# spaceml-org/STARCOP

Measured on AMD Instinct MI355X. Metric: 512x512 hyperspectral tiles/sec (train fwd+bwd), higher is better.
Workload: dtype f32; 1 GPU; configs[1]: HyperSTARCOP U-Net (smp.Unet mobilenet_v2, 4ch mag1c+RGB) train step fwd+loss+bwd+Adam, 512x512 tiles, fp32 HIP kernels (3x3 convs: fp32 operands split exactly into 16-bit terms on the matrix cores, fp32 accumulation; see config.precision and DESIGN.md section 2); batch_per_gpu=16, global_batch=16, parallelism=dp1, hipgraph=False, precision=fp32

## Files before the change

starcop_amd/csrc/conv_bx3.hip:

```cpp
#include "sc_split.h"
#include "conv_sp_pack.h"
#include <cstdlib>
#include <type_traits>


namespace {

struct ConvXP {
  SrcD s0, s1;
  const uintx4* wpk;
  int N, H, W, Cout;
  float* out0; float* out1;
  int csplit, accum0, accum1;
  const float* add0; const float* add1;
  float* stats;
  int down0;
  const float* absmax;
  const float* xb0; const float* xb1;
  int xcdmap;
  const float* bnr_y; const float* bnr_cst; float* bnr_rows; float* bnr_absmax; int bnr_act;
};

static inline void set_bnr(ConvXP& p, const sc_bnr_args* b) {
  p.bnr_y = b ? b->y : nullptr; p.bnr_cst = b ? b->cst : nullptr; p.bnr_rows = b ? b->rows : nullptr;
// ... 1965 lines not shown
      if (nn > nlast) { nn = pn; yy = py; xx = px; }
    };
    if (n1 > nlast) { n1 = n; y1 = y0; x1 = x0; }
    int n2 = n1, y2 = y1, x2 = x1;
    advance_sat(n2, y2, x2);
    if (t_begin < t_end) {
      x_load(xr, n, y0 - 1, x0);
      dy_load(n, y0, x0);
      x_store(xr, y0 - 1, x0, rp);
      x_load(xr, n, y0 + 1, x0);
      dy_store(0, y0, x0);
      x_store(xr, y0 + 1, x0, rp + 2);
      dy_load(n1, y1, x1);
      x_load(xr, n1, y1 + 1, x1);
      __syncthreads();
    }
    for (long t = t_begin; t < t_end; ++t) {
      if (y0 >= 0) compute(rp, buf);
#pragma unroll
      for (int k = 0; k < NDY; ++k) {
        dy_store_item(k, buf ^ 1, y1, x1);
        dy_load_item(k, n2, y2, x2);
      }
#pragma unroll
      for (int k = 0; k < NXI; ++k) {
        x_store_item(xr, k, y1 + 1, x1, rp + 4);
        x_load_item(xr, k, n2, y2 + 1, x2);
      }
      __syncthreads();
      rp = (rp + 2) & 7;
      buf ^= 1;
      n = n1; y0 = y1; x0 = x1;
      n1 = n2; y1 = y2; x1 = x2;
      advance_sat(n2, y2, x2);
    }
  }
  constexpr bool RED = PIPE && (KP == 1 || 3 * NPAIR * 3072 <= NT * CIT * XCP / 2);
  constexpr int KPP = RED ? 1 : KP;
  if constexpr (RED && KP > 1) {
    float* red = reinterpret_cast<float*>(&s_x[0][0]);
    const int slot = pair + NPAIR * kh;
#pragma unroll
    for (int k = 1; k < KP; ++k) {
      if (kp == k) {
#pragma unroll
        for (int kw = 0; kw < 3; ++kw)
#pragma unroll
          for (int r = 0; r < 16; ++r) red[slot * 3072 + (kw * 16 + r) * 64 + lane] = acc[kw][r];
      }
      __syncthreads();
      if (kp == 0) {
#pragma unroll
        for (int kw = 0; kw < 3; ++kw)
#pragma unroll
          for (int r = 0; r < 16; ++r) acc[kw][r] += red[slot * 3072 + (kw * 16 + r) * 64 + lane];
      }
      if (k + 1 < KP) __syncthreads();
    }
    if (kp != 0) return;
  }
  if (NPAIR == 3 && !computing) return;
  const int ci = cit * CIT + wn * 32 + l31;
  const size_t plane = (size_t)p.CoP * p.CiP;
  float* pb = p.part + ((size_t)blockIdx.x * KPP + (RED ? 0 : kp)) * 9 * plane;
#pragma unroll
  for (int kw = 0; kw < 3; ++kw) {
#pragma unroll
    for (int r = 0; r < 16; ++r) {
      const int co = cot * COT + wm * 32 + (r & 3) + 8 * (r >> 2) + 4 * lhi;
      if (co < p.CoP && ci < p.CiP) pb[(kh * 3 + kw) * plane + (size_t)co * p.CiP + ci] = HF ? acc[kw][r] * hinv : acc[kw][r];
    }
  }
}


template <int CIN, bool BNB>
__global__ __launch_bounds__(256, CIN == 32 ? 2 : 3) void k_wgrad_thin_h(const WgradXP p) {
  constexpr int NCB = CIN / 16, SR = 4, RING = 12;
#ifndef SC_WTH_DYPAD
#define SC_WTH_DYPAD(CIN) ((CIN) == 16 ? 16 : 8)
#endif
#ifndef SC_WTH_XPAD
#define SC_WTH_XPAD 16
#endif
  constexpr int DYP = SR * 32 + SC_WTH_DYPAD(CIN);
  constexpr int XP = 40, XCP = RING * XP + SC_WTH_XPAD;
  constexpr int NDY = (16 * SR * 16) / 256;
  constexpr int XCNT = CIN * SR * 17;
  constexpr int NXI = (XCNT + 255) / 256;
  __shared__ __attribute__((aligned(16))) unsigned s_dy[2][2][16 * DYP / 2];
  __shared__ __attribute__((aligned(16))) unsigned s_x[2][CIN * XCP / 2];
  __shared__ __attribute__((aligned(16))) float s_ca[16 * SC_CST];
  __shared__ __attribute__((aligned(16))) float s_cb[CIN * 4];

  const int tid = threadIdx.x, lane = tid & 63, wave = tid >> 6;
  const int l15 = lane & 15, lg = lane >> 4;
  const int H = p.H, W = p.W;
  const float hsg = h_grad_scale(p.absmax);
  const float hsa = h_act_scale(p.xb0, p.xb1);
  const float hinv = 1.f / (hsg * hsa);

  for (int i = tid; i < 16 * SC_CST; i += 256) {
    const int ch = i / SC_CST, f = i % SC_CST;
    const float fs = (BNB ? (f >= 2 && f <= 4) : (f < 2)) ? hsg : 1.f;
    s_ca[i] = fs * ((p.dy.cst && p.dy.mode != SC_SRC_RAW && ch < p.Cout) ? p.dy.cst[(size_t)ch * SC_CST + f] : (f == 0 ? 1.f : 0.f));
  }
  for (int i = tid; i < CIN; i += 256) {
    float sc = 1.f, sh = 0.f;
    if (p.s0.cst && p.s0.mode != SC_SRC_RAW) { sc = p.s0.cst[(size_t)i * SC_CST]; sh = p.s0.cst[(size_t)i * SC_CST + 1]; }
    s_cb[i * 4] = sc * hsa; s_cb[i * 4 + 1] = sh * hsa;
    s_cb[i * 4 + 2] = h_lo(sc_act_lo(p.s0.act), hsa); s_cb[i * 4 + 3] = h_hi(sc_act_hi(p.s0.act), hsa);
  }

  floatx4 acc[9][NCB];
#pragma unroll
  for (int t = 0; t < 9; ++t)
#pragma unroll
    for (int cb = 0; cb < NCB; ++cb) acc[t][cb] = (floatx4){0.f, 0.f, 0.f, 0.f};

  const int tiles_x = (W + 31) >> 5, RS = (H + SR - 1) / SR, RSS = RS + 1;
  const long T = (long)p.N * tiles_x * RSS;
  const long t_begin = T * blockIdx.x / p.nsl, t_end = T * (blockIdx.x + 1) / p.nsl;
  const float dlo = sc_act_lo(p.dy.act) * (BNB ? 1.f : hsg), dhi = sc_act_hi(p.dy.act) * (BNB ? 1.f : hsg);
  const size_t HW = (size_t)H * W;
  const int up = p.s0.up, Ws = W >> up;
  const unsigned istr = (unsigned)((size_t)CIN * (H >> up) * Ws * 4);

  unsigned dyo[NDY], xo[NXI];
#pragma unroll
  for (int k = 0; k < NDY; ++k) {
    const int co = (tid + 256 * k) >> 6;
    dyo[k] = (unsigned)(co < p.Cout ? co : 0) * (unsigned)HW * 4u;
  }
#pragma unroll
  for (int k = 0; k < NXI; ++k) {
    int it = tid + 256 * k;
    if (it >= XCNT) it -= XCNT;
    xo[k] = (unsigned)((it / 17) >> 2) * (unsigned)((H >> up) * Ws) * 4u;
  }

  float dg[NDY][2], dv[BNB ? NDY : 1][2], xr[NXI][2];
  auto dy_load_item = [&](int k, int n, int y0, int x0) {
    const int it = tid + 256 * k;
    const int row = (it >> 4) & 3, col = 2 * (it & 15);
    const int y = y0 + row, x = x0 + col;
    const size_t io = (size_t)n * p.Cout * HW * 4;
    const unsigned off = dyo[k] + (unsigned)(((y >= 0 && y < H) ? y : 0) * W + ((x < W) ? x : 0)) * 4u;
    const float2 g = *reinterpret_cast<const float2*>(reinterpret_cast<const char*>(p.dy.x) + io + off);
    dg[k][0] = g.x; dg[k][1] = g.y;
    if (BNB) {
      const float2 a = *reinterpret_cast<const float2*>(reinterpret_cast<const char*>(p.dy.aux) + io + off);
      dv[k][0] = a.x; dv[k][1] = a.y;
    }
  };
  auto dy_store_item = [&](int k, int buf, int y0, int x0) {
    const int it = tid + 256 * k;
    const int co = it >> 6, row = (it >> 4) & 3, col = 2 * (it & 15);
    const int y = y0 + row, x = x0 + col;
    const bool ok = (co < p.Cout) && y >= 0 && y < H && x < W;
    const float4 c0 = *reinterpret_cast<const float4*>(&s_ca[co * SC_CST]);
    const float c4 = s_ca[co * SC_CST + 4];
    float v0, v1;
    if (BNB) {
      v0 = sc_pro_bnbwd(dg[k][0], dv[k][0], c0.x, c0.y, c0.z, c0.w, c4, dlo, dhi);
      v1 = sc_pro_bnbwd(dg[k][1], dv[k][1], c0.x, c0.y, c0.z, c0.w, c4, dlo, dhi);
    } else {
      v0 = sc_pro_affine(dg[k][0], c0.x, c0.y, dlo, dhi);
      v1 = sc_pro_affine(dg[k][1], c0.x, c0.y, dlo, dhi);
    }
    v0 = ok ? v0 : 0.f;
    v1 = ok ? v1 : 0.f;
    unsigned t0, t1;
    split2h(v0, v1, t0, t1);
    const int d = (co * DYP + row * 32 + col) >> 1;
    s_dy[buf][0][d] = t0; s_dy[buf][1][d] = t1;
  };
  auto x_load_item = [&](int k, int n, int R, int x0) {
    int it = tid + 256 * k;
    if (it >= XCNT) it -= XCNT;
    const int rc = it / 17, pr = it - rc * 17;
    const int rowi = rc & 3;
    const int y = R + rowi, x = x0 - 1 + 2 * pr;
    const int yc = (y >= 0 && y < H) ? y : 0;
    const int xa = (x >= 0 && x < W) ? x : 0, xb = (x + 1 < W) ? x + 1 : 0;
    const char* base = reinterpret_cast<const char*>(p.s0.x) + (size_t)n * istr;
    const unsigned ro = xo[k] + (unsigned)((yc >> up) * Ws) * 4u;
    xr[k][0] = *reinterpret_cast<const float*>(base + (ro + (unsigned)(xa >> up) * 4u));
    xr[k][1] = *reinterpret_cast<const float*>(base + (ro + (unsigned)(xb >> up) * 4u));
  };
  auto x_store_item = [&](int k, int R, int x0, int sl0) {
    int it = tid + 256 * k;
    if (it >= XCNT) it -= XCNT;
    const int rc = it / 17, pr = it - rc * 17;
    const int rowi = rc & 3, cil = rc >> 2;
    const int y = R + rowi, x = x0 - 1 + 2 * pr;
    const bool oky = (y >= 0) && (y < H);
    const float4 c = *reinterpret_cast<const float4*>(&s_cb[cil * 4]);
    float v0 = sc_pro_affine_h(xr[k][0], c.x, c.y, c.z, c.w);
    float v1 = sc_pro_affine_h(xr[k][1], c.x, c.y, c.z, c.w);
    v0 = (oky && x >= 0 && x < W) ? v0 : 0.f;
    v1 = (oky && x + 1 < W) ? v1 : 0.f;
    unsigned t0, t1;
    split2h<false>(v0, v1, t0, t1);
    int slot = sl0 + rowi;
    slot = slot >= RING ? slot - RING : slot;
    const int d = ((cil * XCP + slot * XP) >> 1) + pr;
    s_x[0][d] = t0; s_x[1][d] = t1;
  };
  auto ring = [](int v) { return v >= RING ? v - RING : v; };
  const unsigned opaque_zero = (unsigned)p.H >> 30;
  auto compute = [&](int rp, int buf) {
    const int r = wave;
    halfx8 A[2];
    const int da = (l15 * DYP + r * 32 + 8 * lg) >> 1;
#pragma unroll
    for (int tm = 0; tm < 2; ++tm) A[tm] = __builtin_bit_cast(halfx8, *reinterpret_cast<const uintx4*>(&s_dy[buf][tm][da]));
#pragma unroll
    for (int kh = 0; kh < 3; ++kh) {
      const int slot = ring(rp + r + kh);
#pragma unroll
      for (int cb = 0; cb < NCB; ++cb) {
        const int dx = (((cb * 16 + l15) * XCP + slot * XP) >> 1) + 4 * lg;
        halfx8 B[3][2];
#pragma unroll
        for (int tm = 0; tm < 2; ++tm) {
          const uintx4 X0 = *reinterpret_cast<const uintx4*>(&s_x[tm][dx]);
          const uintx4 X1v = *reinterpret_cast<const uintx4*>(&s_x[tm][dx + 4]);
          const unsigned X1 = X1v[0] | (X1v[1] & opaque_zero);
          uintx4 S1, S2;
          S1[0] = __builtin_amdgcn_alignbit(X0[1], X0[0], 16);
          S1[1] = __builtin_amdgcn_alignbit(X0[2], X0[1], 16);
          S1[2] = __builtin_amdgcn_alignbit(X0[3], X0[2], 16);
          S1[3] = __builtin_amdgcn_alignbit(X1, X0[3], 16);
          S2[0] = X0[1]; S2[1] = X0[2]; S2[2] = X0[3]; S2[3] = X1;
          B[0][tm] = __builtin_bit_cast(halfx8, X0);
          B[1][tm] = __builtin_bit_cast(halfx8, S1);
          B[2][tm] = __builtin_bit_cast(halfx8, S2);
        }
#pragma unroll
        for (int kw = 0; kw < 3; ++kw) {
          floatx4 c = acc[kh * 3 + kw][cb];
          c = __builtin_amdgcn_mfma_f32_16x16x32_f16(A[0], B[kw][1], c, 0, 0, 0);
          c = __builtin_amdgcn_mfma_f32_16x16x32_f16(A[1], B[kw][0], c, 0, 0, 0);
          c = __builtin_amdgcn_mfma_f32_16x16x32_f16(A[0], B[kw][0], c, 0, 0, 0);
          acc[kh * 3 + kw][cb] = c;
        }
      }
    }
  };

  const int nlast = p.N - 1;
  auto advance = [&](int& nn, int& yy, int& xx) {
    const int pn = nn, py = yy, px = xx;
    yy += SR;
    if (yy >= SR * RS) { yy = -SR; xx += 32; if (xx >= 32 * tiles_x) { xx = 0; ++nn; } }
    if (nn > nlast) { nn = pn; yy = py; xx = px; }
  };
  int n = 0, y0 = 0, x0 = 0;
  if (t_begin < t_end) {
    const int strip = (int)(t_begin / RSS), ty = (int)(t_begin - (long)strip * RSS);
    n = strip / tiles_x; x0 = (strip - n * tiles_x) * 32; y0 = (ty - 1) * SR;
  }
  n = __builtin_amdgcn_readfirstlane(n); y0 = __builtin_amdgcn_readfirstlane(y0); x0 = __builtin_amdgcn_readfirstlane(x0);
  int n1 = n, y1 = y0, x1 = x0;
  advance(n1, y1, x1);
  int n2 = n1, y2 = y1, x2 = x1;
  advance(n2, y2, x2);
  __syncthreads();
  int rp = 0, buf = 0;
  if (t_begin < t_end) {
#pragma unroll
    for (int k = 0; k < NXI; ++k) x_load_item(k, n, y0 - 1, x0);
#pragma unroll
    for (int k = 0; k < NDY; ++k) dy_load_item(k, n, y0, x0);
#pragma unroll
    for (int k = 0; k < NXI; ++k) { x_store_item(k, y0 - 1, x0, rp); x_load_item(k, n, y0 + 3, x0); }
#pragma unroll
    for (int k = 0; k < NDY; ++k) { dy_store_item(k, 0, y0, x0); dy_load_item(k, n1, y1, x1); }
#pragma unroll
    for (int k = 0; k < NXI; ++k) { x_store_item(k, y0 + 3, x0, rp + 4); x_load_item(k, n1, y1 + 1, x1); }
    __syncthreads();
  }
  for (long t = t_begin; t < t_end; ++t) {
    if (y0 >= 0) compute(rp, buf);
#pragma unroll
    for (int k = 0; k < NDY; ++k) {
      dy_store_item(k, buf ^ 1, y1, x1);
      dy_load_item(k, n2, y2, x2);
    }
    const int sl1 = ring(rp + 6);
#pragma unroll
    for (int k = 0; k < NXI; ++k) {
      x_store_item(k, y1 + 1, x1, sl1);
      x_load_item(k, n2, y2 + 1, x2);
    }
    __syncthreads();
    rp = ring(rp + 4);
    buf ^= 1;
    n = n1; y0 = y1; x0 = x1;
    n1 = n2; y1 = y2; x1 = x2;
    advance(n2, y2, x2);
  }
  float* red = reinterpret_cast<float*>(&s_x[0][0]);
  auto put = [&](int slot) {
#pragma unroll
    for (int tap = 0; tap < 9; ++tap)
#pragma unroll
      for (int cb = 0; cb < NCB; ++cb)
        *reinterpret_cast<floatx4*>(&red[(((slot * 9 + tap) * NCB + cb) * 64 + lane) * 4]) = acc[tap][cb];
  };
  auto take = [&](int slot) {
#pragma unroll
    for (int tap = 0; tap < 9; ++tap)
#pragma unroll
      for (int cb = 0; cb < NCB; ++cb) acc[tap][cb] += *reinterpret_cast<const floatx4*>(&red[(((slot * 9 + tap) * NCB + cb) * 64 + lane) * 4]);
  };
  if (wave >= 2) put(wave - 2);
  __syncthreads();
  if (wave < 2) take(wave);
  __syncthreads();
  if (wave == 1) put(0);
  __syncthreads();
  if (wave == 0) {
    take(0);
    const size_t plane = (size_t)16 * CIN;
    float* pb = p.part + (size_t)blockIdx.x * 9 * plane;
#pragma unroll
    for (int tap = 0; tap < 9; ++tap)
#pragma unroll
      for (int cb = 0; cb < NCB; ++cb)
#pragma unroll
        for (int r = 0; r < 4; ++r) pb[tap * plane + (size_t)(4 * lg + r) * CIN + cb * 16 + l15] = acc[tap][cb][r] * hinv;
  }
}

struct WgradXPlan { int wm, nci, kp, nsl, CoP, CiP, co_tiles, ci_tiles; };
WgradXPlan plan_wgrad_bx3(int N, int H, int W, int Cout, int Cin, bool allow96 = false) {
  WgradXPlan pl;
  pl.wm = Cout > 32 ? 2 : 1;
  pl.nci = Cin <= 32 ? 1 : 2;
  if (allow96 && pl.wm == 1 && Cin > 64 && Cin <= 96) pl.nci = 3;
  pl.kp = pl.nci * pl.wm == 3 ? 1 : 4 / (pl.nci * pl.wm);
  pl.CoP = (Cout + 31) / 32 * 32;
  pl.CiP = (Cin + 31) / 32 * 32;
  pl.co_tiles = (Cout + 32 * pl.wm - 1) / (32 * pl.wm);
  pl.ci_tiles = (Cin + 32 * pl.nci - 1) / (32 * pl.nci);
  const long T = (long)N * ((W + 31) / 32) * ((H + 1) / 2);
  const long tiles = (long)pl.co_tiles * pl.ci_tiles;
  const long nmax = T / 4 < 512 ? (T / 4 > 1 ? T / 4 : 1) : 512;
  auto cost = [&](long k) { return (double)((tiles * k + 255) / 256) * ((double)((T + k - 1) / k) + 6.0); };
  double best_cost = 1e30;
  for (long k = 1; k <= nmax; ++k) best_cost = cost(k) < best_cost ? cost(k) : best_cost;
  long best = 1;
  for (long k = 1; k <= nmax; ++k)
    if (cost(k) <= 1.03 * best_cost) { best = k; break; }
  long want = best;
  pl.nsl = (int)want;
  return pl;
}


struct PackDesc {
  const float* w; float* wpk;
  int Cout, Cin, ks, co_t, tflip, bx3;
  unsigned long long total;
};
static_assert(sizeof(PackDesc) == sizeof(sc_pack_desc), "sc_pack_desc layout");

__global__ __launch_bounds__(256) void k_pack_batch(const PackDesc* __restrict__ descs, const unsigned* __restrict__ starts, int n) {
  int lo = 0, hi = n - 1;
  while (lo < hi) {
    const int mid = (lo + hi + 1) >> 1;
    if (starts[mid] <= blockIdx.x) lo = mid; else hi = mid - 1;
  }
  const PackDesc d = descs[lo];
  const size_t i = (size_t)(blockIdx.x - starts[lo]) * 256 + threadIdx.x;
  if (i >= d.total) return;
  if (d.bx3 == SC_PACK_THIN16) { pack_thin_item(d.w, reinterpret_cast<unsigned short*>(d.wpk), i, d.Cout, d.Cin, d.tflip); return; }
  if (d.bx3 == SC_PACK_SPD) { spd_pack_item(d.w, reinterpret_cast<unsigned short*>(d.wpk), i, d.Cout, d.Cin, d.co_t, (d.tflip & 3) == 2, (d.tflip & 4) != 0, (d.tflip & 3) == 3 ? d.Cin - d.co_t : 0); return; }
  if (d.bx3 == SC_PACK_SP) { sp_pack_item(d.w, reinterpret_cast<unsigned short*>(d.wpk), i, d.Cout, d.co_t, d.Cin - d.co_t, (d.tflip & 4) != 0); return; }
  const int M = d.tflip ? d.Cin : d.Cout, K = d.tflip ? d.Cout : d.Cin;
  if (d.bx3 == SC_PACK_PW3) {
    const int nks = (K + 15) / 16;
    const int j = (int)(i % 8), lane = (int)((i / 8) % 64);
    const int ks = (int)((i / 512) % nks), cb = (int)(i / ((size_t)512 * nks));
    const int m = cb * 32 + (lane & 31), k = ks * 16 + 8 * (lane >> 5) + j;
    float v = 0.f;
    if (m < M && k < K) v = d.tflip ? d.w[(size_t)k * M + m] : d.w[(size_t)m * K + k];
    unsigned short t[3];
    split_filter(v, false, t);
    unsigned short* out = reinterpret_cast<unsigned short*>(d.wpk);
    for (int c = 0; c < 3; ++c) out[((((size_t)cb * nks + ks) * 3 + c) * 64 + lane) * 8 + j] = t[c];
    return;
  }
  const int taps = d.ks * d.ks;
  if (!d.bx3) {
    const int kc = d.ks == 3 ? 8 : 16;
    const int Kpad = (K + kc - 1) / kc * kc;
    const int col = (int)(i % d.co_t);
    size_t r = i / d.co_t;
    const int tap = (int)(r % taps); r /= taps;
    const int k = (int)(r % Kpad);
    const int m = (int)(r / Kpad) * d.co_t + col;
    float v = 0.f;
    if (m < M && k < K) v = d.tflip ? d.w[((size_t)k * M + m) * taps + (taps - 1 - tap)] : d.w[((size_t)m * K + k) * taps + tap];
    d.wpk[i] = v;
    return;
  }
  const int nchunk = (K + 15) / 16;
  size_t r = i;
  const int j = (int)(r % 8); r /= 8;
  const int col = (int)(r % d.co_t); r /= d.co_t;
  const int half = (int)(r % 2); r /= 2;
  const int kw = (int)(r % 3); r /= 3;
  const int kh = (int)(r % 3); r /= 3;
  const int chunk = (int)(r % nchunk);
  const int mt = (int)(r / nchunk);
  const int m = mt * d.co_t + col, k = chunk * 16 + half * 8 + j, tap = kh * 3 + kw;
  float v = 0.f;
  if (m < M && k < K) v = d.tflip ? d.w[((size_t)k * M + m) * 9 + (8 - tap)] : d.w[((size_t)m * K + k) * 9 + tap];
  unsigned short t[3];
  const bool hmode = d.bx3 == SC_TERMS_F16X2;
  const int nt = hmode ? 2 : d.bx3;
  split_filter(v, hmode, t);
  const size_t stage = ((size_t)mt * nchunk + chunk) * 3 + kh;
  unsigned short* out = reinterpret_cast<unsigned short*>(d.wpk);
  for (int c = 0; c < nt; ++c) out[((((stage * nt + c) * 3 + kw) * 2 + half) * d.co_t + col) * 8 + j] = t[c];
}

}

extern "C" size_t sc_packed_weight_floats_bx3(int Cout, int Cin, int co_t, int transpose_flip, int terms) {
  const int M = transpose_flip ? Cin : Cout, K = transpose_flip ? Cout : Cin;
  const size_t mt = (M + co_t - 1) / co_t, nchunk = (K + 15) / 16;
  return mt * nchunk * 3 * 6 * (size_t)(terms == SC_TERMS_F16X2 ? 2 : (terms >= 1 && terms <= 3 ? terms : 3)) * co_t * 4;
}

extern "C" int sc_pack_weights_bx3(const float* w, float* wpk, int Cout, int Cin, int co_t, int transpose_flip,
                                   int terms, sc_stream stream) {
  SC_REQUIRE(terms >= 1 && terms <= 4, "sc_pack_weights_bx3: terms must be 1, 2, 3 or SC_TERMS_F16X2 (got %d)", terms);
  SC_REQUIRE(w && wpk && Cout > 0 && Cin > 0, "sc_pack_weights_bx3: bad argument");
  SC_REQUIRE(co_t == 32 || co_t == 64, "sc_pack_weights_bx3: co_t must be 32 or 64 (got %d)", co_t);
  SC_REQUIRE(((uintptr_t)wpk & 15) == 0, "sc_pack_weights_bx3: destination must be 16-byte aligned");
  const int M = transpose_flip ? Cin : Cout, K = transpose_flip ? Cout : Cin;
  const int nchunk = (K + 15) / 16;
  const size_t total = (size_t)((M + co_t - 1) / co_t) * nchunk * 9 * 2 * co_t * 8;
  const int blocks = (int)((total + 255) / 256 > 4096 ? 4096 : (total + 255) / 256);
  hipLaunchKernelGGL(k_pack_weights_bx3, dim3(blocks), dim3(256), 0, (hipStream_t)stream, w,
                     reinterpret_cast<unsigned short*>(wpk), Cout, Cin, co_t, transpose_flip, nchunk,
                     terms == SC_TERMS_F16X2 ? 2 : terms, terms == SC_TERMS_F16X2 ? 1 : 0, total);
  SC_LAUNCH_OK("sc_pack_weights_bx3");
  return SC_OK;
}

extern "C" int sc_conv3x3_bx3(const sc_conv_args* a, sc_stream stream) {
  SC_REQUIRE(a != nullptr, "sc_conv3x3_bx3: null args");
  SC_REQUIRE(a->ks == 3, "sc_conv3x3_bx3: ks must be 3 (got %d)", a->ks);
  SC_REQUIRE(a->co_t == 32 || a->co_t == 64, "sc_conv3x3_bx3: co_t must be 32 or 64 (got %d)", a->co_t);
  SC_REQUIRE(a->nsrc == 1 || a->nsrc == 2, "sc_conv3x3_bx3: nsrc must be 1 or 2");
  const int C0 = a->src[0].C, C1 = a->nsrc == 2 ? a->src[1].C : 0;
  SC_REQUIRE(C0 > 0 && C1 >= 0 && (a->nsrc == 1 || (C0 % 16 == 0 && C1 > 0)),
             "sc_conv3x3_bx3: a concat needs the first source's channels to be a multiple of 16 (got %d,%d)", C0, C1);
  SC_REQUIRE(a->N > 0 && a->H > 0 && a->W > 0 && a->Cout > 0, "sc_conv3x3_bx3: bad shape");
  SC_REQUIRE(a->csplit > 0 && a->csplit <= a->Cout, "sc_conv3x3_bx3: bad csplit");
  SC_REQUIRE(a->csplit == a->Cout || (a->add0 == nullptr && a->add1 == nullptr), "sc_conv3x3_bx3: add tensors need a single output");
  SC_REQUIRE(((uintptr_t)a->wpk & 15) == 0, "sc_conv3x3_bx3: packed filters must be 16-byte aligned");
  for (int s = 0; s < a->nsrc; ++s) {
    SC_REQUIRE(a->src[s].up == 0 || (a->H % 2 == 0 && a->W % 2 == 0), "sc_conv3x3_bx3: upsampled source needs even H,W");
    SC_REQUIRE(a->src[s].up == 0 || a->src[s].up == 1, "sc_conv3x3_bx3: up must be 0 or 1");
    SC_REQUIRE(a->src[s].mode == SC_SRC_RAW || a->src[s].cst != nullptr, "sc_conv3x3_bx3: source %d needs constants", s);
    SC_REQUIRE(a->src[s].mode != SC_SRC_NORM, "sc_conv3x3_bx3: NORM sources are the stem's");
    SC_REQUIRE(a->src[s].mode != SC_SRC_BNBWD || a->src[s].aux != nullptr, "sc_conv3x3_bx3: BNBWD source needs aux");
    SC_REQUIRE(a->src[s].mode != SC_SRC_BNBWD || a->nsrc == 1, "sc_conv3x3_bx3: a BNBWD source cannot be part of a concat");
  }
  ConvXP p;
  p.s0 = to_srcd(a->src[0]);
  p.s1 = a->nsrc == 2 ? to_srcd(a->src[1]) : empty_srcd();
  p.wpk = reinterpret_cast<const uintx4*>(a->wpk); p.N = a->N; p.H = a->H; p.W = a->W; p.Cout = a->Cout;
  p.out0 = a->out0; p.out1 = a->out1; p.csplit = a->csplit; p.accum0 = a->accum0; p.accum1 = a->accum1;
  p.add0 = a->add0; p.add1 = a->add1; p.stats = a->stats;
  p.down0 = a->down0 ? 1 : 0;
  SC_REQUIRE(!p.down0 || (a->H % 2 == 0 && a->W % 2 == 0 && a->stats == nullptr && a->add0 == nullptr && a->add1 == nullptr),
             "sc_conv3x3_bx3: down0 (2x2-summed half-resolution out0) needs even H, W and no stats/add tensors");
  const int co_tiles = (a->Cout + a->co_t - 1) / a->co_t;
  dim3 grid(((a->W + 31) / 32) * ((a->H + 7) / 8), co_tiles, a->N);
  constexpr int xcdmap_env = 2;
  p.xcdmap = xcdmap_env >= 2 ? 2 : ((xcdmap_env && co_tiles > 1) ? 1 : 0);
  {
    constexpr long big_env = 0L;
    const long nkc = (C0 + C1 + 15) / 16;
    const long wbytes = (long)co_tiles * nkc * 3 * 6 * (a->terms == SC_TERMS_F16X2 || a->terms == 2 ? 2 : (a->terms == 1 ? 1 : 3)) * a->co_t * 16;
    if (xcdmap_env >= 2 && big_env > 0 && wbytes > big_env && (co_tiles >= 8 || co_tiles == 1 || co_tiles == 2 || co_tiles == 4)) p.xcdmap = 3;
  }
  if (p.xcdmap == 3) {
    const long total = (long)grid.x * a->N;
    const long slots = co_tiles >= 8 ? (long)((co_tiles + 7) / 8) * total : (total + (8 / co_tiles) - 1) / (8 / co_tiles);
    SC_REQUIRE(slots * 8 < (1L << 31), "sc_conv3x3_bx3: grid too large");
    grid = dim3((unsigned)(slots * 8));
  } else if (p.xcdmap) {
    const long pt8 = ((long)grid.x * a->N + 7) / 8 * 8;
    SC_REQUIRE(pt8 * co_tiles < (1L << 31), "sc_conv3x3_bx3: grid too large");
    grid = dim3((unsigned)(pt8 * co_tiles));
  }
  hipStream_t st = (hipStream_t)stream;
  const bool bnb = a->src[0].mode == SC_SRC_BNBWD;
  SC_REQUIRE(a->terms >= 0 && a->terms <= 4, "sc_conv3x3_bx3: terms must be 0 (= 3), 1, 2, 3 or SC_TERMS_F16X2 (got %d)", a->terms);
  p.absmax = a->absmax; p.xb0 = a->xbound[0]; p.xb1 = a->xbound[1];
  set_bnr(p, a->bnr);
  if (a->bnr) {
    SC_REQUIRE(bnb && a->bnr->y && a->bnr->cst && a->bnr->rows, "sc_conv3x3_bx3: bnr needs a BNBWD source and y / cst / rows");
    SC_REQUIRE(!a->accum0 && !a->add0 && !a->add1 && !a->stats, "sc_conv3x3_bx3: bnr: out0 must receive the complete gradient (no accum0 / add / stats)");
    SC_REQUIRE(a->csplit == a->Cout || a->csplit % a->co_t == 0, "sc_conv3x3_bx3: bnr: csplit must fall on a cout-tile boundary");
  }
#define SC_LAUNCH_BX3(NT, HF)                                                                                  \
  do {                                                                                                         \
    if (a->co_t == 64 && bnb) hipLaunchKernelGGL((k_conv3_bx3<2, true, NT, HF>), grid, dim3(256), 0, st, p);   \
    else if (a->co_t == 64) hipLaunchKernelGGL((k_conv3_bx3<2, false, NT, HF>), grid, dim3(256), 0, st, p);    \
    else if (bnb) hipLaunchKernelGGL((k_conv3_bx3<1, true, NT, HF>), grid, dim3(256), 0, st, p);               \
    else hipLaunchKernelGGL((k_conv3_bx3<1, false, NT, HF>), grid, dim3(256), 0, st, p);                       \
  } while (0)
  constexpr int ws_env = 1;
  static const int ws_env_min = [] { const char* e = getenv("STARCOP_BX3_WS_MINCHUNKS"); return e ? atoi(e) : 16; }();
  if (a->terms == 1) SC_LAUNCH_BX3(1, false); else if (a->terms == 2) SC_LAUNCH_BX3(2, false);
  else if (a->terms == SC_TERMS_F16X2 && ws_env && (C0 + C1 + 15) / 16 >= ws_env_min && (!bnb || a->src[0].C <= 256) && !a->bnr) {
    if (a->co_t == 64 && bnb) hipLaunchKernelGGL((k_conv3_ws<2, true>), grid, dim3(512), 0, st, p);
    else if (a->co_t == 64) hipLaunchKernelGGL((k_conv3_ws<2, false>), grid, dim3(512), 0, st, p);
    else if (bnb) hipLaunchKernelGGL((k_conv3_ws<1, true>), grid, dim3(512), 0, st, p);
    else hipLaunchKernelGGL((k_conv3_ws<1, false>), grid, dim3(512), 0, st, p);
  }
  else if (a->terms == SC_TERMS_F16X2) SC_LAUNCH_BX3(2, true); else SC_LAUNCH_BX3(3, false);
#undef SC_LAUNCH_BX3
  SC_LAUNCH_OK("sc_conv3x3_bx3");
  return SC_OK;
}

static bool wgrad3_pipe_reduces(const WgradXPlan& pl) {
  const int npair = pl.nci * pl.wm, cit = 32 * pl.nci, xcp = 8 * 40 + 8;
  return pl.kp == 1 || 3 * npair * 3072 <= 2 * cit * xcp / 2;
}

static size_t wgrad_bx3_workspace_of(const WgradXPlan& pl) {
  const size_t E = (size_t)9 * pl.CoP * pl.CiP;
  const int nparts = pl.nsl * pl.kp;
  return (size_t)nparts * E + sc_reduce_scratch_floats(nparts, E);
}
extern "C" size_t sc_wgrad_bx3_workspace_floats(int N, int H, int W, int Cout, int Cin) {
  const size_t a = wgrad_bx3_workspace_of(plan_wgrad_bx3(N, H, W, Cout, Cin, false));
  const size_t b = wgrad_bx3_workspace_of(plan_wgrad_bx3(N, H, W, Cout, Cin, true));
  return a > b ? a : b;
}

extern "C" int sc_conv3x3_wgrad_bx3(const sc_wgrad_args* a, sc_stream stream) {
  SC_REQUIRE(a != nullptr, "sc_conv3x3_wgrad_bx3: null args");
  SC_REQUIRE(a->ks == 3, "sc_conv3x3_wgrad_bx3: ks must be 3");
  SC_REQUIRE(a->nsrc == 1 || a->nsrc == 2, "sc_conv3x3_wgrad_bx3: nsrc must be 1 or 2");
  const int C0 = a->src[0].C, C1 = a->nsrc == 2 ? a->src[1].C : 0;
  SC_REQUIRE(C0 + C1 == a->Cin, "sc_conv3x3_wgrad_bx3: source channels (%d+%d) != Cin %d", C0, C1, a->Cin);
  SC_REQUIRE(a->dy.C == a->Cout, "sc_conv3x3_wgrad_bx3: dy channels %d != Cout %d", a->dy.C, a->Cout);
  SC_REQUIRE(a->dy.up == 0 && a->dy.mode != SC_SRC_NORM, "sc_conv3x3_wgrad_bx3: unsupported dy source");
  SC_REQUIRE(a->dy.mode != SC_SRC_BNBWD || a->dy.aux != nullptr, "sc_conv3x3_wgrad_bx3: BNBWD dy needs aux");
  SC_REQUIRE(a->N > 0 && a->H > 0 && a->W > 0 && a->Cout > 0 && a->Cin > 0, "sc_conv3x3_wgrad_bx3: bad shape");
  for (int s = 0; s < a->nsrc; ++s) {
    SC_REQUIRE(a->src[s].mode == SC_SRC_RAW || a->src[s].mode == SC_SRC_AFFINE, "sc_conv3x3_wgrad_bx3: input sources must be RAW or AFFINE");
    SC_REQUIRE(a->src[s].up == 0 || (a->src[s].up == 1 && a->H % 2 == 0 && a->W % 2 == 0), "sc_conv3x3_wgrad_bx3: upsampled source needs even H,W");
  }
  static const bool no96 = [] { const char* e = getenv("STARCOP_WGRAD96"); return e && atoi(e) == 0; }();
  constexpr int pipe_env = 1;
  bool pipe = pipe_env && a->terms == SC_TERMS_F16X2 && a->dy.mode == SC_SRC_BNBWD && a->W % 2 == 0 && (((uintptr_t)a->dy.x | (uintptr_t)a->dy.aux) & 7) == 0 &&
              (size_t)a->Cout * a->H * a->W * 4 < (1ull << 32);
  for (int s = 0; s < a->nsrc; ++s) pipe = pipe && (size_t)a->N * a->src[s].C * (a->H >> a->src[s].up) * (a->W >> a->src[s].up) * 4 < (1ull << 32);
  const WgradXPlan pl = plan_wgrad_bx3(a->N, a->H, a->W, a->Cout, a->Cin, pipe && !no96);
  const size_t need = sc_wgrad_bx3_workspace_floats(a->N, a->H, a->W, a->Cout, a->Cin);
  SC_REQUIRE(a->part_floats >= need, "sc_conv3x3_wgrad_bx3: workspace too small (%zu < %zu floats)", a->part_floats, need);
  WgradXP p;
  p.dy = to_srcd(a->dy); p.s0 = to_srcd(a->src[0]); p.s1 = a->nsrc == 2 ? to_srcd(a->src[1]) : empty_srcd();
  p.N = a->N; p.H = a->H; p.W = a->W; p.Cout = a->Cout; p.Cin = a->Cin; p.part = a->part;
  p.nsl = pl.nsl; p.CoP = pl.CoP; p.CiP = pl.CiP;
  dim3 grid(pl.nsl, pl.ci_tiles, pl.co_tiles);
  hipStream_t st = (hipStream_t)stream;
  SC_REQUIRE(a->terms >= 0 && a->terms <= 4, "sc_conv3x3_wgrad_bx3: terms must be 0 (= 3), 1, 2, 3 or SC_TERMS_F16X2 (got %d)", a->terms);
  p.absmax = a->absmax; p.xb0 = a->xbound[0]; p.xb1 = a->xbound[1];
  int nparts = pl.nsl * pl.kp;
#define SC_WGX(WM_, NT_, NCI_, HF_, PIPE_) hipLaunchKernelGGL((k_wgrad3_bx3<WM_, NT_, NCI_, HF_, PIPE_>), grid, dim3(768), 0, st, p)
#define SC_WGX_NT(NT_, HF_, PIPE_)                                   \
  do {                                                               \
    if constexpr (HF_ && PIPE_) { if (pl.nci == 3) { SC_WGX(1, NT_, 3, HF_, PIPE_); break; } }      \
    if (pl.wm == 2 && pl.nci == 2) SC_WGX(2, NT_, 2, HF_, PIPE_);    \
    else if (pl.wm == 2) SC_WGX(2, NT_, 1, HF_, PIPE_);              \
    else if (pl.nci == 2) SC_WGX(1, NT_, 2, HF_, PIPE_);             \
    else SC_WGX(1, NT_, 1, HF_, PIPE_);                              \
  } while (0)
  if (a->terms == 1) SC_WGX_NT(1, false, false); else if (a->terms == 2) SC_WGX_NT(2, false, false);
  else if (a->terms == SC_TERMS_F16X2) {
    if (pipe) { SC_WGX_NT(2, true, true); if (wgrad3_pipe_reduces(pl)) nparts = pl.nsl; } else SC_WGX_NT(2, true, false);
  }
  else SC_WGX_NT(3, false, false);
#undef SC_WGX_NT
#undef SC_WGX
  SC_LAUNCH_OK("sc_conv3x3_wgrad_bx3");
  return sc_wgrad_finish(a->part, nparts, 9, a->Cout, a->Cin, pl.CoP, pl.CiP, a->dw, st);
}

static int wgrad_thin16_slices(int N, int H, int W, int Cin) {
  const long T = (long)N * ((W + 31) / 32) * ((H + 3) / 4 + 1);
  const long full = Cin > 16 ? 512 : 768;
  return (int)(T < full ? T : full);
}

extern "C" size_t sc_wgrad_thin16_workspace_floats(int N, int H, int W, int Cout, int Cin) {
  (void)Cout;
  const size_t E = (size_t)9 * 16 * Cin;
  const int nparts = wgrad_thin16_slices(N, H, W, Cin);
  return (size_t)nparts * E + sc_reduce_scratch_floats(nparts, E);
}

extern "C" int sc_conv3x3_wgrad_thin16(const sc_wgrad_args* a, sc_stream stream) {
  SC_REQUIRE(a != nullptr && a->ks == 3 && a->nsrc == 1, "sc_conv3x3_wgrad_thin16: one source, ks = 3");
  SC_REQUIRE(a->Cout >= 1 && a->Cout <= 16 && (a->Cin == 16 || a->Cin == 32) && a->src[0].C == a->Cin && a->dy.C == a->Cout,
             "sc_conv3x3_wgrad_thin16: needs <= 16 output and 16 or 32 input channels (got %d, %d)", a->Cout, a->Cin);
  SC_REQUIRE(a->N > 0 && a->H > 0 && a->W > 0, "sc_conv3x3_wgrad_thin16: bad shape");
  SC_REQUIRE(a->terms == SC_TERMS_F16X2, "sc_conv3x3_wgrad_thin16: terms must be SC_TERMS_F16X2");
  SC_REQUIRE(a->dy.up == 0 && a->dy.mode != SC_SRC_NORM && (a->dy.mode != SC_SRC_BNBWD || a->dy.aux != nullptr), "sc_conv3x3_wgrad_thin16: unsupported dy source");
  SC_REQUIRE(a->dy.mode == SC_SRC_RAW || a->dy.cst != nullptr, "sc_conv3x3_wgrad_thin16: dy source needs constants");
  const sc_src& s = a->src[0];
  SC_REQUIRE((s.mode == SC_SRC_RAW || (s.mode == SC_SRC_AFFINE && s.cst != nullptr)), "sc_conv3x3_wgrad_thin16: input source must be RAW or AFFINE");
  SC_REQUIRE(s.up == 0 || (s.up == 1 && a->H % 2 == 0 && a->W % 2 == 0), "sc_conv3x3_wgrad_thin16: upsampled source needs even H, W");
  SC_REQUIRE((size_t)a->Cout * a->H * a->W * 4 < (1ull << 32) && (size_t)a->N * a->Cin * a->H * a->W * 4 < (1ull << 32),
             "sc_conv3x3_wgrad_thin16: tensors too large for 32-bit byte offsets");
  SC_REQUIRE(a->W % 2 == 0 && (((uintptr_t)a->dy.x | (uintptr_t)a->dy.aux) & 7) == 0, "sc_conv3x3_wgrad_thin16: needs an even width and 8-byte aligned gradient tensors");
  const size_t need = sc_wgrad_thin16_workspace_floats(a->N, a->H, a->W, a->Cout, a->Cin);
  SC_REQUIRE(a->part_floats >= need, "sc_conv3x3_wgrad_thin16: workspace too small (%zu < %zu floats)", a->part_floats, need);
  WgradXP p;
  p.absmax = a->absmax; p.xb0 = a->xbound[0]; p.xb1 = a->xbound[1];
  p.dy = to_srcd(a->dy); p.s0 = to_srcd(s); p.s1 = empty_srcd();
  p.N = a->N; p.H = a->H; p.W = a->W; p.Cout = a->Cout; p.Cin = a->Cin; p.part = a->part;
  p.nsl = wgrad_thin16_slices(a->N, a->H, a->W, a->Cin); p.CoP = 16; p.CiP = a->Cin;
  hipStream_t st = (hipStream_t)stream;
  const bool bnb = a->dy.mode == SC_SRC_BNBWD;
  dim3 grid(p.nsl);
  if (a->Cin == 16) { if (bnb) hipLaunchKernelGGL((k_wgrad_thin_h<16, true>), grid, dim3(256), 0, st, p); else hipLaunchKernelGGL((k_wgrad_thin_h<16, false>), grid, dim3(256), 0, st, p); }
  else              { if (bnb) hipLaunchKernelGGL((k_wgrad_thin_h<32, true>), grid, dim3(256), 0, st, p); else hipLaunchKernelGGL((k_wgrad_thin_h<32, false>), grid, dim3(256), 0, st, p); }
  SC_LAUNCH_OK("sc_conv3x3_wgrad_thin16");
  return sc_wgrad_finish(a->part, p.nsl, 9, a->Cout, a->Cin, 16, a->Cin, a->dw, st);
}

static int thin_steps(int Cout, int Cin, int transpose_flip) {
  const int K = transpose_flip ? Cout : Cin;
  if (transpose_flip && Cin == 32) return 16;
  return (9 * (K / 8) + 3) / 4 + ((!transpose_flip && K == 32) ? 16 : 0);
}

extern "C" size_t sc_packed_weight_floats_thin16(int Cout, int Cin, int transpose_flip) {
  return (size_t)thin_steps(Cout, Cin, transpose_flip) * 2 * 64 * 4;
}

static bool thin16_shape_ok(int Cout, int Cin, int transpose_flip) {
  const int M = transpose_flip ? Cin : Cout, K = transpose_flip ? Cout : Cin;
  if (transpose_flip && Cin == 32 && Cout == 16) return true;
  return M >= 1 && M <= 16 && (K == 16 || K == 32);
}

extern "C" int sc_pack_weights_thin16(const float* w, float* wpk, int Cout, int Cin, int transpose_flip, sc_stream stream) {
  SC_REQUIRE(w && wpk && ((uintptr_t)wpk & 15) == 0, "sc_pack_weights_thin16: bad pointer");
  SC_REQUIRE(thin16_shape_ok(Cout, Cin, transpose_flip), "sc_pack_weights_thin16: needs <= 16 output and 16 or 32 input channels (got %d, %d, flip %d)",
             Cout, Cin, transpose_flip);
  const size_t total = (size_t)thin_steps(Cout, Cin, transpose_flip) * 512;
  hipLaunchKernelGGL(k_pack_weights_thin, dim3((unsigned)((total + 255) / 256)), dim3(256), 0, (hipStream_t)stream, w,
                     reinterpret_cast<unsigned short*>(wpk), Cout, Cin, transpose_flip, total);
  SC_LAUNCH_OK("sc_pack_weights_thin16");
  return SC_OK;
}

extern "C" int sc_conv3x3_thin16(const sc_conv_args* a, sc_stream stream) {
  SC_REQUIRE(a != nullptr && a->ks == 3 && a->nsrc == 1, "sc_conv3x3_thin16: one source, ks = 3");
  const int Cin = a->src[0].C;
  if (a->down0) {
    const sc_src& s = a->src[0];
    SC_REQUIRE(Cin == 16 && a->Cout == 32 && a->csplit == 32 && s.mode == SC_SRC_BNBWD && s.aux && s.cst && s.up == 0,
               "sc_conv3x3_thin16(down0): needs a 16-channel BatchNorm-backward source and 32 output channels (got %d, %d)", Cin, a->Cout);
    SC_REQUIRE(a->H % 2 == 0 && a->W % 2 == 0 && a->N > 0 && a->N <= 65535 && a->out0 && !a->add0 && !a->add1 && !a->stats && !a->bnr && !a->out1,
               "sc_conv3x3_thin16(down0): even H, W; one output, no add / statistics / bnr epilogue");
    SC_REQUIRE(a->terms == SC_TERMS_F16X2 && ((uintptr_t)a->wpk & 15) == 0, "sc_conv3x3_thin16(down0): terms must be SC_TERMS_F16X2, filters 16-byte aligned");
    SC_REQUIRE((size_t)16 * a->H * a->W < ((size_t)1 << 30), "sc_conv3x3_thin16(down0): one image of the gradient must stay below 2^30 elements");
    ConvXP p{};
    p.s0 = to_srcd(s); p.s1 = empty_srcd();
    p.wpk = reinterpret_cast<const uintx4*>(a->wpk); p.N = a->N; p.H = a->H; p.W = a->W; p.Cout = a->Cout;
    p.out0 = a->out0; p.csplit = a->Cout; p.accum0 = a->accum0; p.absmax = a->absmax;
    set_bnr(p, nullptr);
    const long total = (long)((a->W + 63) / 64) * ((a->H + 7) / 8) * a->N, per_xcd = (total + 7) / 8;
    p.xcdmap = 2;
    hipLaunchKernelGGL(k_conv3_thin_spd, dim3((unsigned)(per_xcd * 8)), dim3(256), 0, (hipStream_t)stream, p);
    SC_LAUNCH_OK("sc_conv3x3_thin16(down0)");
    return SC_OK;
  }
  SC_REQUIRE(a->Cout >= 1 && a->Cout <= 16 && (Cin == 16 || Cin == 32), "sc_conv3x3_thin16: needs <= 16 output and 16 or 32 input channels (got %d, %d)",
             a->Cout, Cin);
  SC_REQUIRE(a->N > 0 && a->N <= 65535 && a->H > 0 && a->W > 0, "sc_conv3x3_thin16: bad shape");
  SC_REQUIRE(a->csplit == a->Cout && !a->accum0 && !a->add0 && !a->add1 && !a->down0 && a->out0,
             "sc_conv3x3_thin16: a single plain output only (no split / add / accumulate / down-sum epilogue)");
  SC_REQUIRE(a->terms == SC_TERMS_F16X2, "sc_conv3x3_thin16: terms must be SC_TERMS_F16X2");
  SC_REQUIRE(((uintptr_t)a->wpk & 15) == 0, "sc_conv3x3_thin16: packed filters must be 16-byte aligned");
  const sc_src& s = a->src[0];
  SC_REQUIRE(s.up == 0 || (s.up == 1 && a->H % 2 == 0 && a->W % 2 == 0), "sc_conv3x3_thin16: upsampled source needs even H, W");
  SC_REQUIRE(s.mode == SC_SRC_RAW || s.cst != nullptr, "sc_conv3x3_thin16: source needs constants");
  SC_REQUIRE(s.mode != SC_SRC_NORM && (s.mode != SC_SRC_BNBWD || s.aux != nullptr), "sc_conv3x3_thin16: unsupported source");
  SC_REQUIRE((size_t)a->Cout * a->H * a->W < ((size_t)1 << 30), "sc_conv3x3_thin16: one image of the output must stay below 2^30 elements");
  ConvXP p{};
  p.s0 = to_srcd(s); p.s1 = empty_srcd();
  p.wpk = reinterpret_cast<const uintx4*>(a->wpk); p.N = a->N; p.H = a->H; p.W = a->W; p.Cout = a->Cout;
  p.out0 = a->out0; p.csplit = a->Cout; p.stats = a->stats; p.absmax = a->absmax; p.xb0 = a->xbound[0]; p.xb1 = a->xbound[1];
  set_bnr(p, a->bnr);
  SC_REQUIRE(!a->bnr || (s.mode == SC_SRC_BNBWD && a->bnr->y && a->bnr->cst && a->bnr->rows && !a->stats),
             "sc_conv3x3_thin16: bnr needs a BNBWD source, y / cst / rows and no stats");
  static const bool sp_off = [] { const char* e = getenv("STARCOP_THIN_SP"); return e && atoi(e) == 0; }();
  const bool thin_sp = Cin == 32 && s.up == 1 && s.mode != SC_SRC_BNBWD && !sp_off;
  const int tw = (Cin == 16 || thin_sp) ? 64 : 32;
  dim3 grid(((a->W + tw - 1) / tw) * ((a->H + 7) / 8), 1, a->N);
  constexpr int xcdmap_env = 2;
  p.xcdmap = xcdmap_env ? 2 : 0;
  if (p.xcdmap) {
    const long total = (long)grid.x * a->N, per_xcd = (total + 7) / 8;
    grid = dim3((unsigned)(per_xcd * 8));
  }
  hipStream_t st = (hipStream_t)stream;
  const bool bnb = s.mode == SC_SRC_BNBWD;
  static const bool ups_off = [] { const char* e = getenv("STARCOP_THIN_UPS"); return e && atoi(e) == 0; }();
  if (thin_sp) hipLaunchKernelGGL(k_conv3_thin_sp, grid, dim3(256), 0, st, p);
  else if (Cin == 16) { if (bnb) hipLaunchKernelGGL((k_conv3_thin_h<16, true>), grid, dim3(256), 0, st, p); else hipLaunchKernelGGL((k_conv3_thin_h<16, false>), grid, dim3(256), 0, st, p); }
  else if (s.up == 1 && !bnb && !ups_off) hipLaunchKernelGGL((k_conv3_thin_h<32, false, true>), grid, dim3(256), 0, st, p);
  else           { if (bnb) hipLaunchKernelGGL((k_conv3_thin_h<32, true>), grid, dim3(256), 0, st, p); else hipLaunchKernelGGL((k_conv3_thin_h<32, false>), grid, dim3(256), 0, st, p); }
  SC_LAUNCH_OK("sc_conv3x3_thin16");
  return SC_OK;
}

extern "C" size_t sc_pack_work_items(int Cout, int Cin, int ks, int co_t, int transpose_flip, int bx3) {
  if (bx3 == SC_PACK_THIN16) return (size_t)thin_steps(Cout, Cin, transpose_flip) * 512;
  if (bx3 == SC_PACK_SPD) return spd_pack_items(Cout, co_t, (transpose_flip & 3) == 3 ? Cin - co_t : 0);
  if (bx3 == SC_PACK_SP) return sp_pack_items(Cout, co_t, Cin - co_t);
  if (bx3 == SC_PACK_PW3) {
    const int M = transpose_flip ? Cin : Cout, K = transpose_flip ? Cout : Cin;
    return (size_t)(((M + 31) / 32 + 3) / 4 * 4) * ((K + 15) / 16) * 512;
  }
  if (bx3) {
    const int M = transpose_flip ? Cin : Cout, K = transpose_flip ? Cout : Cin;
    return (size_t)((M + co_t - 1) / co_t) * ((K + 15) / 16) * 9 * 2 * co_t * 8;
  }
  return sc_packed_weight_floats(Cout, Cin, ks, co_t, transpose_flip);
}

extern "C" int sc_pack_weights_batch(const sc_pack_desc* descs_dev, const uint32_t* block_starts_dev, int n, uint32_t total_blocks,
                                     sc_stream stream) {
  SC_REQUIRE(descs_dev && block_starts_dev && n > 0 && total_blocks > 0, "sc_pack_weights_batch: bad argument");
  hipLaunchKernelGGL(k_pack_batch, dim3(total_blocks), dim3(256), 0, (hipStream_t)stream,
                     reinterpret_cast<const PackDesc*>(descs_dev), block_starts_dev, n);
  SC_LAUNCH_OK("sc_pack_weights_batch");
  return SC_OK;
}
```

Baseline: 1446 tiles/s.

## Add specialized wgrad kernel for 2x-upsampled 32-channel thin convs

Adds k_wgrad_thin_sp, a weight-gradient kernel for 3x3 convs whose input is a 2x nearest-upsampled 32-channel source. It reads the input at low resolution and pre-sums 2x2 blocks of dy per tap, so each upsampled input pixel is multiplied once instead of four times. The MFMA work per tile shrinks and the input is never materialised at high resolution. It is selected by default for even H/W with Cin=32 and up=1, can be disabled via env vars, and the workspace sizing is extended to match.

Result: no change. 1459 tiles/s, median of 6 (+0.9%).

```diff
diff --git a/starcop_amd/csrc/conv_bx3.hip b/starcop_amd/csrc/conv_bx3.hip
--- a/starcop_amd/csrc/conv_bx3.hip
+++ b/starcop_amd/csrc/conv_bx3.hip
@@ -2291,6 +2291,257 @@
     advance(n2, y2, x2);
   }
   float* red = reinterpret_cast<float*>(&s_x[0][0]);
+  auto put = [&](int slot) {
+#pragma unroll
+    for (int tap = 0; tap < 9; ++tap)
+#pragma unroll
+      for (int cb = 0; cb < NCB; ++cb)
+        *reinterpret_cast<floatx4*>(&red[(((slot * 9 + tap) * NCB + cb) * 64 + lane) * 4]) = acc[tap][cb];
+  };
+  auto take = [&](int slot) {
+#pragma unroll
+    for (int tap = 0; tap < 9; ++tap)
+#pragma unroll
+      for (int cb = 0; cb < NCB; ++cb) acc[tap][cb] += *reinterpret_cast<const floatx4*>(&red[(((slot * 9 + tap) * NCB + cb) * 64 + lane) * 4]);
+  };
+  if (wave >= 2) put(wave - 2);
+  __syncthreads();
+  if (wave < 2) take(wave);
+  __syncthreads();
+  if (wave == 1) put(0);
+  __syncthreads();
+  if (wave == 0) {
+    take(0);
+    const size_t plane = (size_t)16 * CIN;
+    float* pb = p.part + (size_t)blockIdx.x * 9 * plane;
+#pragma unroll
+    for (int tap = 0; tap < 9; ++tap)
+#pragma unroll
+      for (int cb = 0; cb < NCB; ++cb)
+#pragma unroll
+        for (int r = 0; r < 4; ++r) pb[tap * plane + (size_t)(4 * lg + r) * CIN + cb * 16 + l15] = acc[tap][cb][r] * hinv;
+  }
+}
+
+template <bool BNB>
+__global__ __launch_bounds__(256, 2) void k_wgrad_thin_sp(const WgradXP p) {
+  constexpr int CIN = 32, NCB = 2, RING = 10, DP = 68, DCP = RING * DP + 4;
+  constexpr int XCP = 4 * 32 + 16;
+  __shared__ __attribute__((aligned(16))) float s_d[16 * DCP];
+  __shared__ __attribute__((aligned(16))) unsigned s_x[2][CIN * XCP / 2];
+  __shared__ __attribute__((aligned(16))) float s_ca[16 * SC_CST];
+  __shared__ __attribute__((aligned(16))) float s_cb[CIN * 4];
+  static_assert(2 * 9 * NCB * 256 <= 16 * DCP, "the wave reduction reuses the dy ring");
+
+  const int tid = threadIdx.x, lane = tid & 63, wave = tid >> 6;
+  const int l15 = lane & 15, lg = lane >> 4;
+  const int H = p.H, W = p.W, Hl = H >> 1, Wl = W >> 1;
+  const float hsg = h_grad_scale<3>(p.absmax);
+  const float hsa = h_act_scale(p.xb0, p.xb1);
+  const float hinv = 1.f / (hsg * hsa);
+
+  for (int i = tid; i < 16 * SC_CST; i += 256) {
+    const int ch = i / SC_CST, f = i % SC_CST;
+    const float fs = (BNB ? (f >= 2 && f <= 4) : (f < 2)) ? hsg : 1.f;
+    s_ca[i] = fs * ((p.dy.cst && p.dy.mode != SC_SRC_RAW && ch < p.Cout) ? p.dy.cst[(size_t)ch * SC_CST + f] : (f == 0 ? 1.f : 0.f));
+  }
+  for (int i = tid; i < CIN; i += 256) {
+    float sc = 1.f, sh = 0.f;
+    if (p.s0.cst && p.s0.mode != SC_SRC_RAW) { sc = p.s0.cst[(size_t)i * SC_CST]; sh = p.s0.cst[(size_t)i * SC_CST + 1]; }
+    s_cb[i * 4] = sc * hsa; s_cb[i * 4 + 1] = sh * hsa;
+    s_cb[i * 4 + 2] = h_lo(sc_act_lo(p.s0.act), hsa); s_cb[i * 4 + 3] = h_hi(sc_act_hi(p.s0.act), hsa);
+  }
+
+  floatx4 acc[9][NCB];
+#pragma unroll
+  for (int t = 0; t < 9; ++t)
+#pragma unroll
+    for (int cb = 0; cb < NCB; ++cb) acc[t][cb] = (floatx4){0.f, 0.f, 0.f, 0.f};
+
+  const int tiles_x = (Wl + 31) >> 5, RS = (Hl + 3) >> 2, RSS = RS + 1;
+  const long T = (long)p.N * tiles_x * RSS;
+  const int t_begin = (int)(T * blockIdx.x / p.nsl), t_end = (int)(T * (blockIdx.x + 1) / p.nsl);
+  const float dlo = sc_act_lo(p.dy.act) * (BNB ? 1.f : hsg), dhi = sc_act_hi(p.dy.act) * (BNB ? 1.f : hsg);
+  const unsigned HW4 = (unsigned)(H * W) * 4u, HWl4 = (unsigned)(Hl * Wl) * 4u;
+
+  const int drow = tid >> 5, dpair = tid & 31;
+  const int fco = tid >> 4, frow = (tid >> 1) & 7, fside = tid & 1;
+  const int xci = tid >> 6, xrow = (tid >> 4) & 3, xpr = tid & 15;
+  struct Item { int n, s, tx, minrow; };
+  auto item_of = [&](int t, int minrow) {
+    Item it;
+    const int strip = t / RSS;
+    it.s = t - strip * RSS - 1;
+    it.n = strip / tiles_x;
+    it.tx = strip - it.n * tiles_x;
+    it.minrow = minrow;
+    return it;
+  };
+
+  float dg[16][2], dv[BNB ? 16 : 1][2], fg, fv = 0.f, xr[8][2];
+  auto load = [&](const Item& it) {
+    const size_t io = (size_t)it.n * p.Cout * HW4;
+    const char* gb = reinterpret_cast<const char*>(p.dy.x) + io;
+    const char* ab = BNB ? reinterpret_cast<const char*>(p.dy.aux) + io : nullptr;
+    {
+      const int y = 8 * it.s + 1 + drow, x = 64 * it.tx + 2 * dpair;
+      const bool ok = drow >= it.minrow && y >= 0 && y < H && x < W;
+      const unsigned off = ok ? (unsigned)(y * W + x) * 4u : 0u;
+#pragma unroll
+      for (int k = 0; k < 16; ++k) {
+        const unsigned o = off + (k < p.Cout ? (unsigned)k * HW4 : 0u);
+        const float2 g = *reinterpret_cast<const float2*>(gb + o);
+        dg[k][0] = g.x; dg[k][1] = g.y;
+        if constexpr (BNB) {
+          const float2 a = *reinterpret_cast<const float2*>(ab + o);
+          dv[k][0] = a.x; dv[k][1] = a.y;
+        }
+      }
+    }
+    {
+      const int y = 8 * it.s + 1 + frow, x = 64 * it.tx + (fside ? 64 : -1);
+      const bool ok = fco < p.Cout && frow >= it.minrow && y >= 0 && y < H && x >= 0 && x < W;
+      const unsigned o = ok ? (unsigned)fco * HW4 + (unsigned)(y * W + x) * 4u : 0u;
+      fg = *reinterpret_cast<const float*>(gb + o);
+      if constexpr (BNB) fv = *reinterpret_cast<const float*>(ab + o);
+    }
+    {
+      const int i = 4 * it.s + xrow, j = 32 * it.tx + 2 * xpr;
+      const bool oky = it.minrow == 0 && i >= 0 && i < Hl;
+      const char* xb = reinterpret_cast<const char*>(p.s0.x) + (size_t)it.n * CIN * HWl4;
+      const unsigned o0 = (oky && j < Wl) ? (unsigned)(i * Wl + j) * 4u : 0u;
+      const unsigned o1 = (oky && j + 1 < Wl) ? (unsigned)(i * Wl + j + 1) * 4u : 0u;
+#pragma unroll
+      for (int k = 0; k < 8; ++k) {
+        const unsigned c = (unsigned)(xci + 4 * k) * HWl4;
+        xr[k][0] = *reinterpret_cast<const float*>(xb + (c + o0));
+        xr[k][1] = *reinterpret_cast<const float*>(xb + (c + o1));
+      }
+    }
+  };
+  auto ring = [](int v) { return v >= RING ? v - RING : v; };
+  auto store = [&](const Item& it, int rb) {
+    {
+      const int y = 8 * it.s + 1 + drow, x = 64 * it.tx + 2 * dpair;
+      const bool ok = drow >= it.minrow && y >= 0 && y < H && x < W;
+      float* dst = &s_d[ring(rb + drow) * DP + 2 + 2 * dpair];
+#pragma unroll
+      for (int k = 0; k < 16; ++k) {
+        const float4 c0 = *reinterpret_cast<const float4*>(&s_ca[k * SC_CST]);
+        float v0, v1;
+        if constexpr (BNB) {
+          const float c4 = s_ca[k * SC_CST + 4];
+          v0 = sc_pro_bnbwd(dg[k][0], dv[k][0], c0.x, c0.y, c0.z, c0.w, c4, dlo, dhi);
+          v1 = sc_pro_bnbwd(dg[k][1], dv[k][1], c0.x, c0.y, c0.z, c0.w, c4, dlo, dhi);
+        } else {
+          v0 = sc_pro_affine(dg[k][0], c0.x, c0.y, dlo, dhi);
+          v1 = sc_pro_affine(dg[k][1], c0.x, c0.y, dlo, dhi);
+        }
+        const bool okk = ok && k < p.Cout;
+        *reinterpret_cast<float2*>(dst + k * DCP) = make_float2(okk ? v0 : 0.f, okk ? v1 : 0.f);
+      }
+    }
+    {
+      const int y = 8 * it.s + 1 + frow, x = 64 * it.tx + (fside ? 64 : -1);
+      const bool ok = fco < p.Cout && frow >= it.minrow && y >= 0 && y < H && x >= 0 && x < W;
+      const float4 c0 = *reinterpret_cast<const float4*>(&s_ca[fco * SC_CST]);
+      float v;
+      if constexpr (BNB) v = sc_pro_bnbwd(fg, fv, c0.x, c0.y, c0.z, c0.w, s_ca[fco * SC_CST + 4], dlo, dhi);
+      else v = sc_pro_affine(fg, c0.x, c0.y, dlo, dhi);
+      s_d[fco * DCP + ring(rb + frow) * DP + (fside ? 66 : 1)] = ok ? v : 0.f;
+    }
+    {
+      const int i = 4 * it.s + xrow, j = 32 * it.tx + 2 * xpr;
+      const bool oky = it.minrow == 0 && i >= 0 && i < Hl;
+      const bool ok0 = oky && j < Wl, ok1 = oky && j + 1 < Wl;
+#pragma unroll
+      for (int k = 0; k < 8; ++k) {
+        const int ci = xci + 4 * k;
+        const float4 c = *reinterpret_cast<const float4*>(&s_cb[ci * 4]);
+        float v0 = sc_pro_affine_h(xr[k][0], c.x, c.y, c.z, c.w);
+        float v1 = sc_pro_affine_h(xr[k][1], c.x, c.y, c.z, c.w);
+        v0 = ok0 ? v0 : 0.f;
+        v1 = ok1 ? v1 : 0.f;
+        unsigned t0, t1;
+        split2h<false>(v0, v1, t0, t1);
+        const int d = ((ci * XCP + xrow * 32) >> 1) + xpr;
+        s_x[0][d] = t0; s_x[1][d] = t1;
+      }
+    }
+  };
+  auto compute = [&](int rb) {
+    halfx8 B[NCB][2];
+#pragma unroll
+    for (int cb = 0; cb < NCB; ++cb)
+#pragma unroll
+      for (int tm = 0; tm < 2; ++tm)
+        B[cb][tm] = __builtin_bit_cast(halfx8, *reinterpret_cast<const uintx4*>(&s_x[tm][(((cb * 16 + l15) * XCP + wave * 32) >> 1) + 4 * lg]));
+    float d[4][18];
+#pragma unroll
+    for (int r = 0; r < 4; ++r) {
+      int slot = rb + 2 * wave - 2 + r;
+      slot = slot < 0 ? slot + RING : ring(slot);
+      const float* rp = &s_d[l15 * DCP + slot * DP + 16 * lg];
+      d[r][0] = rp[1];
+      const float2 a = *reinterpret_cast<const float2*>(rp + 2);
+      d[r][1] = a.x; d[r][2] = a.y;
+#pragma unroll
+      for (int q = 0; q < 3; ++q) {
+        const float4 b = *reinterpret_cast<const float4*>(rp + 4 + 4 * q);
+        d[r][3 + 4 * q] = b.x; d[r][4 + 4 * q] = b.y; d[r][5 + 4 * q] = b.z; d[r][6 + 4 * q] = b.w;
+      }
+      const float2 e = *reinterpret_cast<const float2*>(rp + 16);
+      d[r][15] = e.x; d[r][16] = e.y;
+      d[r][17] = rp[18];
+    }
+#pragma unroll
+    for (int kh = 0; kh < 3; ++kh) {
+      float rs[18];
+#pragma unroll
+      for (int c = 0; c < 18; ++c) rs[c] = d[2 - kh][c] + d[3 - kh][c];
+#pragma unroll
+      for (int kw = 0; kw < 3; ++kw) {
+        uintx4 a0, a1;
+#pragma unroll
+        for (int j = 0; j < 4; ++j) {
+          const float s0 = rs[4 * j + 2 - kw] + rs[4 * j + 3 - kw];
+          const float s1 = rs[4 * j + 4 - kw] + rs[4 * j + 5 - kw];
+          unsigned t0, t1;
+          split2h(s0, s1, t0, t1);
+          a0[j] = t0; a1[j] = t1;
+        }
+        const halfx8 A0 = __builtin_bit_cast(halfx8, a0), A1 = __builtin_bit_cast(halfx8, a1);
+#pragma unroll
+        for (int cb = 0; cb < NCB; ++cb) {
+          floatx4 c = acc[kh * 3 + kw][cb];
+          c = __builtin_amdgcn_mfma_f32_16x16x32_f16(A0, B[cb][1], c, 0, 0, 0);
+          c = __builtin_amdgcn_mfma_f32_16x16x32_f16(A1, B[cb][0], c, 0, 0, 0);
+          c = __builtin_amdgcn_mfma_f32_16x16x32_f16(A0, B[cb][0], c, 0, 0, 0);
+          acc[kh * 3 + kw][cb] = c;
+        }
+      }
+    }
+  };
+
+  __syncthreads();
+  if (t_begin < t_end) {
+    const int first = t_begin - (item_of(t_begin, 0).s >= 0 ? 1 : 0);
+    Item cur = item_of(first, 6);
+    load(cur);
+    int rb = 0;
+    for (int t = first; t < t_end; ++t) {
+      store(cur, rb);
+      __builtin_amdgcn_sched_barrier(0);
+      const Item nxt = item_of(t + 1 < t_end ? t + 1 : t, 0);
+      load(nxt);
+      __syncthreads();
+      if (t != first && cur.s >= 0) compute(rb);
+      __syncthreads();
+      rb = ring(rb + 8);
+      cur = nxt;
+    }
+  }
+  float* red = s_d;
   auto put = [&](int slot) {
 #pragma unroll
     for (int tap = 0; tap < 9; ++tap)
@@ -2596,10 +2847,21 @@
   return (int)(T < full ? T : full);
 }
 
+static int wgrad_thin_sp_slices(int N, int H, int W) {
+  const long T = (long)N * ((W / 2 + 31) / 32) * ((H / 2 + 3) / 4 + 1);
+  static const int cap = [] { const char* e = getenv("STARCOP_THIN_SPW_SLICES"); const int v = e ? atoi(e) : 0; return v >= 1 && v < 512 ? v : 512; }();
+  return (int)(T < cap ? T : cap);
+}
+static bool wgrad_thin_sp_takes(int H, int W, int Cin, int up) {
+  static const bool spw_off = [] { const char* e = getenv("STARCOP_THIN_SPW"); return e && atoi(e) == 0; }();
+  return !spw_off && up == 1 && Cin == 32 && H % 2 == 0 && W % 2 == 0;
+}
+
 extern "C" size_t sc_wgrad_thin16_workspace_floats(int N, int H, int W, int Cout, int Cin) {
   (void)Cout;
   const size_t E = (size_t)9 * 16 * Cin;
-  const int nparts = wgrad_thin16_slices(N, H, W, Cin);
+  int nparts = wgrad_thin16_slices(N, H, W, Cin);
+  if (Cin == 32 && H % 2 == 0 && W % 2 == 0) { const int nsp = wgrad_thin_sp_slices(N, H, W); nparts = nsp > nparts ? nsp : nparts; }
   return (size_t)nparts * E + sc_reduce_scratch_floats(nparts, E);
 }
 
@@ -2626,6 +2888,12 @@
   p.nsl = wgrad_thin16_slices(a->N, a->H, a->W, a->Cin); p.CoP = 16; p.CiP = a->Cin;
   hipStream_t st = (hipStream_t)stream;
   const bool bnb = a->dy.mode == SC_SRC_BNBWD;
+  if (wgrad_thin_sp_takes(a->H, a->W, a->Cin, s.up)) {
+    p.nsl = wgrad_thin_sp_slices(a->N, a->H, a->W);
+    if (bnb) hipLaunchKernelGGL((k_wgrad_thin_sp<true>), dim3(p.nsl), dim3(256), 0, st, p); else hipLaunchKernelGGL((k_wgrad_thin_sp<false>), dim3(p.nsl), dim3(256), 0, st, p);
+    SC_LAUNCH_OK("sc_conv3x3_wgrad_thin16");
+    return sc_wgrad_finish(a->part, p.nsl, 9, a->Cout, a->Cin, 16, a->Cin, a->dw, st);
+  }
   dim3 grid(p.nsl);
   if (a->Cin == 16) { if (bnb) hipLaunchKernelGGL((k_wgrad_thin_h<16, true>), grid, dim3(256), 0, st, p); else hipLaunchKernelGGL((k_wgrad_thin_h<16, false>), grid, dim3(256), 0, st, p); }
   else              { if (bnb) hipLaunchKernelGGL((k_wgrad_thin_h<32, true>), grid, dim3(256), 0, st, p); else hipLaunchKernelGGL((k_wgrad_thin_h<32, false>), grid, dim3(256), 0, st, p); }
```
